# pinterest/rocksplicator

Hardware: AMD Instinct MI355X
Metric: replicated updates/sec (Put+Delete) at 1024 shards (higher is better)
Workload: dtype u8; 1 GPU; 1024shards_16Bkey_1024Bval_zipf0.99; key_len=16, val_len=1024, tick_updates=819200, parallelism=shard-parallel x1

## Files before the change

### rocksplicator_amd/csrc/engine.hip

```cpp
#include <hip/hip_runtime.h>

#define WB_UNALIGNED_OK 1

#include <algorithm>
#include <atomic>
#include <chrono>
#include <cstdio>
#include <cstring>
#include <deque>
#include <map>
#include <memory>
#include <mutex>
#include <string>
#include <thread>
#include <vector>

#include "../../include/rocksplicator_gpu.h"
#include "fold.h"
#include "host_store.h"
#include "part_copy.h"
#include "snappy.h"
#include "wb_format.h"

static thread_local std::string g_err;
extern "C" const char *gra_last_error(void) { return g_err.c_str(); }

#define HIP_TRY(x)                                                     \
  do {                                                                 \
    hipError_t _e = (x);                                               \
    if (_e != hipSuccess) {                                            \
      g_err = std::string(#x) + ": " + hipGetErrorString(_e);          \
      return GRA_ERR;                                                  \
    }                                                                  \
  } while (0)

namespace gra {

struct UpdDesc {
  uint64_t off;
  uint64_t base_seq;
  uint32_t len;
  uint32_t shard;
};
struct TickPlace {
  uint64_t cur;
  uint64_t hdr_off;
  uint64_t payload_off;
  uint64_t payload_bytes;
  uint32_t total_rec;
  uint32_t overflow;
};
struct SnapTask {
  uint64_t comp_off;
  uint64_t out_off;
  uint32_t comp_len;
  uint32_t ulen;
};
struct GroupDesc {
  uint32_t shard, first, n_upds, _pad;
};
struct DevRunDesc {
  uint64_t base_seq, last_seq;
  uint64_t cur;
  uint64_t hdr_off, payload_off;
  uint32_t n_entries, payload_bytes;
  uint32_t pay_rel_base;
  uint32_t shard;
};

__host__ __device__ inline uint2 add2(uint2 a, uint2 b) {
  return make_uint2(a.x + b.x, a.y + b.y);
}


constexpr uint32_t kSnapStage = 508;

__global__ void __launch_bounds__(256) k_snappy(
    const uint8_t *__restrict__ comp, const SnapTask *__restrict__ tasks,
    uint32_t n, uint8_t *__restrict__ scratch,
    uint32_t *__restrict__ err_ring, uint32_t tick) {
  __shared__ uint8_t lds[256 * (kSnapStage + 4)];
  uint32_t i = blockIdx.x * blockDim.x + threadIdx.x;
  if (i >= n) return;
  SnapTask t = tasks[i];
  uint8_t *dst = scratch + t.out_off;
  uint32_t r;
  if (t.comp_len <= kSnapStage) {
    uint8_t *mine = lds + threadIdx.x * (kSnapStage + 4);
    const uint8_t *src = comp + t.comp_off;
    for (uint32_t b = 0; b < t.comp_len; b += 16)
      *(uint4 *)(mine + b) = *(const uint4 *)(src + b);
    r = snp::decompress(mine, t.comp_len, dst, t.ulen);
  } else {
    r = snp::decompress(comp + t.comp_off, t.comp_len, dst, t.ulen);
  }
  if (r != t.ulen) {
    for (int b = 0; b < 13; b++) dst[b] = 0xFF;
    atomicAdd(&err_ring[tick % 64u], 1u);
  }
}

constexpr uint32_t kErrRing = 64;

constexpr uint32_t kRecCache = 2;

__device__ __forceinline__ uint2 block_scan256(uint2 v, uint2 *total) {
  __shared__ uint2 wsum[4];
  const uint32_t lane = threadIdx.x & 63u, w = threadIdx.x >> 6;
  uint2 inc = v;
  for (int ofs = 1; ofs < 64; ofs <<= 1) {
    uint32_t x = __shfl_up(inc.x, ofs, 64), y = __shfl_up(inc.y, ofs, 64);
    if (lane >= (uint32_t)ofs) inc = add2(inc, make_uint2(x, y));
  }
  if (lane == 63) wsum[w] = inc;
  __syncthreads();
  uint2 before = make_uint2(0, 0), tot = make_uint2(0, 0);
  for (uint32_t k = 0; k < 4; k++) {
    uint2 s = wsum[k];
    if (k < w) before = add2(before, s);
    tot = add2(tot, s);
  }
  *total = tot;
  return make_uint2(before.x + inc.x - v.x, before.y + inc.y - v.y);
}

__global__ void k_decode(const uint8_t *__restrict__ blobs,
                         const UpdDesc *__restrict__ descs, uint32_t n,
                         wb::WalkTotals *__restrict__ totals, uint32_t max_rec,
                         uint32_t *__restrict__ err_ring, uint32_t tick,
                         uint2 *__restrict__ partial, uint2 *__restrict__ bsums,
                         wb::Rec *__restrict__ reccache,
                         uint8_t *__restrict__ ok_out) {
  uint32_t i = blockIdx.x * 256 + threadIdx.x;
  uint2 v = make_uint2(0, 0);
  if (i < n) {
    UpdDesc d = descs[i];
    wb::Rec *cache = reccache + (size_t)i * kRecCache;
    wb::WalkTotals t = wb::walk_f(blobs + d.off, d.len,
                                  [&](const wb::Rec &r, uint32_t idx) {
                                    if (idx < kRecCache) cache[idx] = r;
                                  });
    if (t.n_records > max_rec) t.ok = 0;
    totals[i] = t;
    ok_out[i] = (uint8_t)t.ok;
    if (!t.ok) atomicAdd(&err_ring[tick % kErrRing], 1u);
    if (t.ok) v = make_uint2(t.n_records, t.payload16);
  }
  uint2 tot;
  uint2 excl = block_scan256(v, &tot);
  if (i < n) partial[i] = excl;
  if (threadIdx.x == 255) bsums[blockIdx.x] = tot;
}

__global__ void k_scan2(uint2 *__restrict__ bsums, uint32_t nblocks,
                        uint64_t *__restrict__ cursor,
                        TickPlace *__restrict__ place, uint64_t cap, int ring,
                        uint32_t task_cap, uint32_t *__restrict__ err_ring,
                        uint32_t tick) {
  const uint32_t per = (nblocks + 255) / 256;
  const uint32_t lo = threadIdx.x * per < nblocks ? threadIdx.x * per : nblocks;
  const uint32_t hi = lo + per < nblocks ? lo + per : nblocks;
  uint2 mine = make_uint2(0, 0);
  for (uint32_t i = lo; i < hi; i++) mine = add2(mine, bsums[i]);
  uint2 carry;
  uint2 run = block_scan256(mine, &carry);
  for (uint32_t i = lo; i < hi; i++) {
    uint2 v = bsums[i];
    bsums[i] = run;
    run = add2(run, v);
  }
  if (threadIdx.x == 0) {
    bsums[nblocks] = carry;
    uint2 tot = carry;
    uint64_t need_hdr = (((uint64_t)tot.x * sizeof(wb::RecHdr)) + 15) & ~15ULL;
    uint64_t need_pay = tot.y;
    uint64_t need = need_hdr + need_pay;
    TickPlace p = {};
    p.total_rec = tot.x;
    p.payload_bytes = need_pay;
    uint64_t cur = *cursor;
    if ((cur % cap) + need > cap) cur += cap - (cur % cap);
    if (need > cap || (!ring && cur + need > cap) ||
        (uint64_t)tot.x * 2 > task_cap) {
      p.overflow = 1;
      p.total_rec = 0;
      atomicAdd(&err_ring[tick % kErrRing], 1u);
    } else {
      p.cur = cur;
      p.hdr_off = cur % cap;
      p.payload_off = (cur % cap) + need_hdr;
      *cursor = cur + need;
    }
    *place = p;
    err_ring[(tick + kErrRing / 2) % kErrRing] = 0;
  }
}

__global__ void k_emit(const uint8_t *__restrict__ blobs,
                       const UpdDesc *__restrict__ descs, uint32_t n,
                       const wb::WalkTotals *__restrict__ totals,
                       const uint2 *__restrict__ partial,
                       const uint2 *__restrict__ bsums,
                       const TickPlace *__restrict__ place,
                       uint8_t *__restrict__ store,
                       CopyTask *__restrict__ tasks,
                       const wb::Rec *__restrict__ reccache) {
  uint32_t i = blockIdx.x * blockDim.x + threadIdx.x;
  if (i >= n) return;
  if (place->overflow) return;
  wb::WalkTotals t = totals[i];
  if (!t.ok || t.n_records == 0) return;
  UpdDesc d = descs[i];
  uint2 base = add2(partial[i], bsums[i >> 8]);
  wb::RecHdr *hdrs = (wb::RecHdr *)(store + place->hdr_off);
  uint8_t *pay_region = store + place->payload_off;
  uint32_t pay = base.y;
  uint32_t rec = base.x;
  auto emit_one = [&](const wb::Rec &r, uint32_t idx) {
    uint32_t cf4 = r.cf_id ? 4u : 0u;
    uint8_t btag = wb::base_tag(r.tag);
    uint32_t cfv = (cf4 && btag == wb::kRangeDeletion) ? 4u : 0u;
    wb::RecHdr h;
    h.seq = d.base_seq + idx;
    h.kv_off = pay;
    h.val_len = r.val_len + cfv;
    h.key_len = (uint16_t)(r.key_len + cf4);
    h.type = btag;
    h.flags = cf4 ? 1 : 0;
    h.kpref = 0;
    hdrs[rec + idx] = h;
    if (cf4) {
      *(uint32_t *)(pay_region + pay) = r.cf_id;
    }
    CopyTask tk;
    tk.src_off = d.off + r.key_off;
    tk.dst_rel = pay + cf4;
    tk.nbytes = r.key_len;
    tasks[2 * (rec + idx)] = tk;
    if (cfv) {
      uint8_t *p = pay_region + pay + cf4 + r.key_len;
      p[0] = (uint8_t)r.cf_id;
      p[1] = (uint8_t)(r.cf_id >> 8);
      p[2] = (uint8_t)(r.cf_id >> 16);
      p[3] = (uint8_t)(r.cf_id >> 24);
    }
    tk.src_off = d.off + r.val_off;
    tk.dst_rel = pay + cf4 + r.key_len + cfv;
    tk.nbytes = r.val_len;
    tasks[2 * (rec + idx) + 1] = tk;
    pay += (cf4 + r.key_len + cfv + r.val_len + 15u) & ~15u;
  };
  if (t.n_records <= kRecCache) {
    const wb::Rec *cache = reccache + (size_t)i * kRecCache;
    for (uint32_t idx = 0; idx < t.n_records; idx++) emit_one(cache[idx], idx);
  } else {
    wb::walk_f(blobs + d.off, d.len, emit_one);
  }
}

template <int G>
__device__ __forceinline__ void copy_dword(uint8_t *dst, const uint8_t *src,
                                           uint32_t n, uint32_t lane) {
  uint32_t head = (uint32_t)((0u - (uint32_t)(uintptr_t)dst) & 3u);
  if (head > n) head = n;
  if (lane < head) dst[lane] = src[lane];
  dst += head;
  src += head;
  n -= head;
  uint32_t nw = n >> 2;
  uint32_t r = (uint32_t)((uintptr_t)src & 3);
  const uint32_t *asrc = (const uint32_t *)(src - r);
  uint32_t *adst = (uint32_t *)dst;
  if (r == 0) {
    for (uint32_t w = lane; w < nw; w += G) adst[w] = asrc[w];
  } else {
    uint32_t sh = 8 * r;
    for (uint32_t w = lane; w < nw; w += G)
      adst[w] = (asrc[w] >> sh) | (asrc[w + 1] << (32 - sh));
  }
  uint32_t done = nw << 2, tail = n & 3;
  if (lane < tail) dst[done + lane] = src[done + lane];
}

template <int G, int R, bool UNAL>
__global__ void __launch_bounds__(256) k_copy(const uint8_t *__restrict__ blobs,
                                              uint8_t *__restrict__ store,
                                              const TickPlace *__restrict__ place,
                                              const CopyTask *__restrict__ tasks) {
  if (place->overflow) return;
  uint32_t wave = (blockIdx.x * blockDim.x + threadIdx.x) >> 6;
  uint32_t nwaves = (gridDim.x * blockDim.x) >> 6;
  pcopy::part_copy<G, R, UNAL>(blobs, store + place->payload_off, tasks,
                               place->total_rec, wave, nwaves);
}

__global__ void k_drain(const uint8_t *__restrict__ store,
                        const TickPlace *__restrict__ place,
                        uint8_t *__restrict__ hostbuf) {
  if (place->overflow) return;
  uint64_t hdr_bytes = (uint64_t)place->total_rec * sizeof(wb::RecHdr);
  uint64_t hb16 = (hdr_bytes + 15) & ~15ull;
  uint64_t pay = place->payload_bytes;
  const uint8_t *hsrc = store + place->hdr_off;
  const uint8_t *psrc = store + place->payload_off;
  size_t stride = (size_t)gridDim.x * blockDim.x * 16;
  size_t i0 = ((size_t)blockIdx.x * blockDim.x + threadIdx.x) * 16;
  for (size_t b = i0; b < hdr_bytes; b += stride)
    *(uint4 *)(hostbuf + b) = *(const uint4 *)(hsrc + b);
  uint8_t *pdst = hostbuf + hb16;
  for (size_t b = i0; b < pay; b += stride)
    *(uint4 *)(pdst + b) = *(const uint4 *)(psrc + b);
}

__global__ void k_rundesc(const GroupDesc *__restrict__ groups, uint32_t ngroups,
                          const UpdDesc *__restrict__ descs,
                          const wb::WalkTotals *__restrict__ totals,
                          const uint2 *__restrict__ partial,
                          const uint2 *__restrict__ bsums, uint32_t n,
                          uint32_t nblocks,
                          const TickPlace *__restrict__ place,
                          DevRunDesc *__restrict__ out) {
  uint32_t g = blockIdx.x * blockDim.x + threadIdx.x;
  if (g >= ngroups) return;
  GroupDesc gd = groups[g];
  auto scan_at = [&](uint32_t j) {
    return j >= n ? bsums[nblocks] : add2(partial[j], bsums[j >> 8]);
  };
  uint2 s0 = scan_at(gd.first);
  uint2 s1 = scan_at(gd.first + gd.n_upds);
  DevRunDesc rd = {};
  rd.shard = gd.shard;
  rd.n_entries = s1.x - s0.x;
  rd.payload_bytes = s1.y - s0.y;
  rd.pay_rel_base = s0.y;
  if (!place->overflow) {
    rd.cur = place->cur;
    rd.hdr_off = place->hdr_off + (uint64_t)s0.x * sizeof(wb::RecHdr);
    rd.payload_off = place->payload_off + s0.y;
    rd.base_seq = descs[gd.first].base_seq;
    const UpdDesc last = descs[gd.first + gd.n_upds - 1];
    rd.last_seq = last.base_seq + totals[gd.first + gd.n_upds - 1].hdr_count - 1;
  } else {
    rd.n_entries = 0;
  }
  out[g] = rd;
}

struct RunView {
  uint64_t hdr_off, payload_off;
  uint32_t n_entries, pay_rel_base;
};

__device__ inline int dev_memcmp(const uint8_t *a, const uint8_t *b, uint32_t n) {
  for (uint32_t i = 0; i < n; i++) {
    if (a[i] != b[i]) return a[i] < b[i] ? -1 : 1;
  }
  return 0;
}

struct MgExtra {
  uint64_t term_seq, merge_seq, rd_seq;
  uint32_t term_type, _pad;
};

__global__ void k_multiget(const uint8_t *__restrict__ store,
                           const RunView *__restrict__ runs, uint32_t nruns,
                           const GraKeyRef *__restrict__ keys,
                           const uint8_t *__restrict__ keybuf, uint32_t nq,
                           uint8_t *__restrict__ valbuf, uint32_t val_stride,
                           GraGetResult *__restrict__ out,
                           MgExtra *__restrict__ extra, int fold_u64) {
  __shared__ uint64_t sh_term_seq[256];
  __shared__ uint64_t sh_term_ref[256];
  __shared__ uint64_t sh_merge_seq[256];
  __shared__ uint64_t sh_rd_seq[256];
  uint32_t q = blockIdx.x;
  if (q >= nq) return;
  const uint8_t *key = keybuf + keys[q].off;
  uint32_t klen = keys[q].len;
  uint32_t qpref = wb::key_fnv_fold(wb::kFnvBasis32, key, klen);
  uint64_t term_seq = 0, term_ref = ~0ULL, merge_seq = 0, rd_seq = 0;
  for (uint32_t r = 0; r < nruns; r++) {
    RunView rv = runs[r];
    const wb::RecHdr *hdrs = (const wb::RecHdr *)(store + rv.hdr_off);
    const uint8_t *pay = store + rv.payload_off;
    for (uint32_t i = threadIdx.x; i < rv.n_entries; i += blockDim.x) {
      wb::RecHdr h = hdrs[i];
      if (h.type != wb::kRangeDeletion &&
          (h.key_len != klen || h.kpref != qpref))
        continue;
      uint32_t rel = h.kv_off - rv.pay_rel_base;
      if (h.type == wb::kRangeDeletion) {
        const uint8_t *b = pay + rel, *e2 = pay + rel + h.key_len;
        uint32_t bl = h.key_len, el = h.val_len;
        int c1 = dev_memcmp(b, key, bl < klen ? bl : klen);
        if (c1 > 0 || (c1 == 0 && bl > klen)) continue;
        int c2 = dev_memcmp(key, e2, klen < el ? klen : el);
        if (c2 > 0 || (c2 == 0 && klen >= el)) continue;
        if (h.seq > rd_seq) rd_seq = h.seq;
        continue;
      }
      if (dev_memcmp(pay + rel, key, klen) != 0)
        continue;
      if (h.type == wb::kMerge) {
        if (h.seq > merge_seq) merge_seq = h.seq;
      } else if (h.seq > term_seq) {
        term_seq = h.seq;
        term_ref = ((uint64_t)r << 32) | i;
      }
    }
  }
  uint32_t tid = threadIdx.x;
  sh_term_seq[tid] = term_seq;
  sh_term_ref[tid] = term_ref;
  sh_merge_seq[tid] = merge_seq;
  sh_rd_seq[tid] = rd_seq;
  __syncthreads();
  for (uint32_t ofs = blockDim.x / 2; ofs > 0; ofs >>= 1) {
    if (tid < ofs) {
      if (sh_term_seq[tid + ofs] > sh_term_seq[tid]) {
        sh_term_seq[tid] = sh_term_seq[tid + ofs];
        sh_term_ref[tid] = sh_term_ref[tid + ofs];
      }
      if (sh_merge_seq[tid + ofs] > sh_merge_seq[tid])
        sh_merge_seq[tid] = sh_merge_seq[tid + ofs];
      if (sh_rd_seq[tid + ofs] > sh_rd_seq[tid])
        sh_rd_seq[tid] = sh_rd_seq[tid + ofs];
    }
    __syncthreads();
  }
  uint64_t T = sh_term_seq[0], M = sh_merge_seq[0], RD = sh_rd_seq[0];
  uint64_t ref = sh_term_ref[0];
  uint8_t term_type = 0xFF;
  wb::RecHdr h = {};
  RunView rv = {};
  if (ref != ~0ULL) {
    rv = runs[ref >> 32];
    h = ((const wb::RecHdr *)(store + rv.hdr_off))[(uint32_t)ref];
    term_type = h.type;
  }
  if (tid == 0 && extra) {
    extra[q].term_seq = T;
    extra[q].merge_seq = M;
    extra[q].rd_seq = RD;
// ... 594 lines not shown
hipEvent_t GraEngine::get_event() {
  if (!event_pool.empty()) {
    hipEvent_t e = event_pool.back();
    event_pool.pop_back();
    return e;
  }
  hipEvent_t e;
  (void)hipEventCreate(&e);
  return e;
}
void GraEngine::put_event(hipEvent_t e) { event_pool.push_back(e); }

int GraEngine::init(const GraEngineOpts &o) {
  opts = o;
  if (opts.store_bytes == 0) opts.store_bytes = 4ULL << 30;
  if (opts.staging_bytes == 0) opts.staging_bytes = 256ULL << 20;
  if (opts.max_wb_records == 0) opts.max_wb_records = 1024;
  max_upd = 1u << 20;
  task_cap = 4u << 20;
  copy_grid = 2048;
  if (const char *g = getenv("GRA_COPY_GRID")) {
    long v = atol(g);
    copy_grid = (uint32_t)(v < 1 ? 1 : v > 2048 ? 2048 : v);
  }
  group_cap = opts.nshards + 1 > 65536 ? opts.nshards + 1 : 65536;
  (void)hipGetLastError();
  int ndev = 0;
  hipError_t de = hipGetDeviceCount(&ndev);
  if (de != hipSuccess || ndev == 0) {
    g_err = "no HIP device present — the GPU apply path refuses to run "
            "(no CPU fallback by design)";
    return GRA_NO_GPU;
  }
  if (opts.device >= 0) {
    hipError_t se = hipSetDevice(opts.device);
    if (se != hipSuccess) {
      g_err = std::string("hipSetDevice: ") + hipGetErrorString(se);
      (void)hipGetLastError();
      return GRA_ERR;
    }
  }
  HIP_TRY(hipStreamCreate(&stream));
  HIP_TRY(hipStreamCreate(&copyout));
  HIP_TRY(hipStreamCreate(&h2d));
  HIP_TRY(hipStreamCreate(&prep));
  HIP_TRY(hipMalloc(&d_store, opts.store_bytes + 16));
  HIP_TRY(hipMalloc(&d_cursor, 8));
  HIP_TRY(hipMemset(d_cursor, 0, 8));
  HIP_TRY(hipMalloc(&d_totals, (size_t)max_upd * sizeof(wb::WalkTotals)));
  HIP_TRY(hipMalloc(&d_partial, (size_t)max_upd * sizeof(uint2)));
  HIP_TRY(hipMalloc(&d_bsums, ((size_t)max_upd / 256 + 2) * sizeof(uint2)));
  HIP_TRY(hipMalloc(&d_reccache, (size_t)max_upd * 2 * sizeof(wb::Rec)));
  HIP_TRY(hipMalloc(&d_tasks, (size_t)task_cap * sizeof(CopyTask)));
  HIP_TRY(hipMalloc(&d_place, kSlots * sizeof(TickPlace)));
  HIP_TRY(hipMalloc(&d_groups, (size_t)group_cap * sizeof(GroupDesc)));
  HIP_TRY(hipMalloc(&d_err_ring, kErrRing * 4));
  HIP_TRY(hipMemset(d_err_ring, 0, kErrRing * 4));
  for (int i = 0; i < 2; i++) {
    HIP_TRY(hipMalloc(&d_stage_blobs_bufs[i], opts.staging_bytes + 16));
    HIP_TRY(hipMalloc(&d_stage_descs_bufs[i], (size_t)max_upd * sizeof(UpdDesc)));
    HIP_TRY(hipEventCreate(&stage_used_ev[i]));
    HIP_TRY(hipEventRecord(stage_used_ev[i], stream));
    HIP_TRY(hipEventCreateWithFlags(&h2d_gate_ev[i], hipEventDisableTiming));
    HIP_TRY(hipEventRecord(h2d_gate_ev[i], h2d));
  }
  static std::atomic<uint64_t> g_epoch{1};
  for (int i = 0; i < 2; i++) {
    HIP_TRY(hipHostMalloc(&stage[i].pin, opts.staging_bytes + 16,
                          hipHostMallocNonCoherent));
    stage[i].descs = (GraUpdateDesc *)malloc((size_t)max_upd * sizeof(GraUpdateDesc));
    stage[i].epoch = g_epoch.fetch_add(1u << 20);
    HIP_TRY(hipEventCreate(&stage[i].free_ev));
    HIP_TRY(hipEventRecord(stage[i].free_ev, stream));
  }
  cur_stage.store(&stage[0]);
  for (int i = 0; i < kSlots; i++) {
    Slot &s = slots[i];
    HIP_TRY(hipHostMalloc(&s.h_groups, (size_t)group_cap * sizeof(GroupDesc)));
    HIP_TRY(hipHostMalloc(&s.h_place, sizeof(TickPlace)));
    HIP_TRY(hipHostMalloc(&s.h_rundescs, (size_t)group_cap * sizeof(DevRunDesc)));
    HIP_TRY(hipMalloc(&s.d_rundescs, (size_t)group_cap * sizeof(DevRunDesc)));
    HIP_TRY(hipMalloc(&s.d_ok, (size_t)max_upd));
    HIP_TRY(hipHostMalloc(&s.h_ok, (size_t)max_upd));
    HIP_TRY(hipHostMalloc(&s.h_err, 4));
    HIP_TRY(hipHostMalloc(&s.h_descs, (size_t)max_upd * sizeof(UpdDesc)));
  }
  if (opts.drain_host && opts.store_ring &&
      opts.store_bytes < 10 * opts.staging_bytes) {
    g_err = "drain_host with store_ring needs store_bytes >= 10x "
            "staging_bytes (ring wrap inside the drain pipeline)";
    return GRA_ERR;
  }
  shards = std::vector<ShardState>(opts.nshards);
  event_pool.reserve(kSlots * kEventsPerTick);
  for (int i = 0; i < kSlots * kEventsPerTick; i++) {
    hipEvent_t ev;
    HIP_TRY(hipEventCreate(&ev));
    event_pool.push_back(ev);
  }
  return GRA_OK;
}

GraEngine::~GraEngine() {
  {
    std::lock_guard<std::mutex> lk(drain_mu);
    closing = true;
  }
  (void)hipStreamSynchronize(stream);
  (void)hipStreamSynchronize(copyout);
  (void)hipStreamSynchronize(h2d);
  for (auto &t : pending)
    for (int i = 0; i < kEventsPerTick; i++)
      if (t.ev[i]) (void)hipEventDestroy(t.ev[i]);
  for (auto e : event_pool) (void)hipEventDestroy(e);
  for (int i = 0; i < 2; i++) {
    if (stage[i].pin) (void)hipHostFree(stage[i].pin);
    free(stage[i].descs);
    if (stage[i].free_ev) (void)hipEventDestroy(stage[i].free_ev);
  }
  for (int i = 0; i < kSlots; i++) {
    Slot &s = slots[i];
    if (s.h_groups) (void)hipHostFree(s.h_groups);
    if (s.h_place) (void)hipHostFree(s.h_place);
    if (s.h_rundescs) (void)hipHostFree(s.h_rundescs);
    if (s.d_rundescs) (void)hipFree(s.d_rundescs);
    if (s.d_ok) (void)hipFree(s.d_ok);
    if (s.h_ok) (void)hipHostFree(s.h_ok);
    if (s.h_err) (void)hipHostFree(s.h_err);
    if (s.h_descs) (void)hipHostFree(s.h_descs);
  }
  for (void *p : {(void *)mg.d_runs, (void *)mg.d_keys, (void *)mg.d_keybuf,
                  (void *)mg.d_valbuf, (void *)mg.d_out, mg.d_extra,
                  mg.d_qtab, mg.d_cands, mg.d_tombs, mg.d_aux,
                  (void *)mg.d_counts})
    if (p) (void)hipFree(p);
  if (mg.h_counts) (void)hipHostFree(mg.h_counts);
  for (void *p : {(void *)sc.d_runs, (void *)sc.d_bounds, (void *)sc.d_out,
                  (void *)sc.d_cands, (void *)sc.d_tombs, (void *)sc.d_items,
                  (void *)sc.d_bsums, (void *)sc.d_ents, (void *)sc.d_ctl,
                  (void *)sc.d_heads, (void *)sc.d_folds, (void *)sc.d_cp})
    if (p) (void)hipFree(p);
  if (sc.h_ctl) (void)hipHostFree(sc.h_ctl);
  if (sc.h_cp) (void)hipHostFree(sc.h_cp);
  for (int i = 0; i < 2; i++) {
    if (d_stage_blobs_bufs[i]) (void)hipFree(d_stage_blobs_bufs[i]);
    if (d_stage_descs_bufs[i]) (void)hipFree(d_stage_descs_bufs[i]);
    if (stage_used_ev[i]) (void)hipEventDestroy(stage_used_ev[i]);
    if (h2d_gate_ev[i]) (void)hipEventDestroy(h2d_gate_ev[i]);
  }
  for (void *p : {(void *)d_totals, (void *)d_partial, (void *)d_bsums,
                  (void *)d_reccache, (void *)d_store, (void *)d_cursor,
                  (void *)d_tasks,
                  (void *)d_place, (void *)d_groups, (void *)d_err_ring})
    if (p) (void)hipFree(p);
  shards.clear();
  pending.clear();
  {
    std::lock_guard<std::mutex> lk(drain_mu);
    for (auto &pr : drain_pool) (void)hipHostFree(pr.first);
    drain_pool.clear();
  }
  if (stream) (void)hipStreamDestroy(stream);
  if (copyout) (void)hipStreamDestroy(copyout);
  if (h2d) (void)hipStreamDestroy(h2d);
  if (prep) (void)hipStreamDestroy(prep);
}

int GraEngine::free_slot() {
  for (;;) {
    for (int i = 0; i < kSlots; i++)
      if (!slots[i].busy) return i;
    int rc = ingest(false);
    if (rc != GRA_OK) return -1;
    if (!pending.empty()) {
      if (ingest_one(pending.front(), true) != GRA_OK) return -1;
      pending.pop_front();
    }
  }
}

int GraEngine::enqueue_tick(TickInput &in) {
  const uint32_t n = in.n;
  const uint64_t blob_bytes = in.blob_bytes;
  const std::vector<GroupDesc> &groups = *in.groups;
  if (n == 0) return GRA_OK;
  if (n > max_upd) {
    g_err = "tick exceeds max updates per tick";
    return GRA_ERR;
  }
  if (opts.drain_host && opts.store_ring && blob_bytes * 10 > opts.store_bytes) {
    g_err = "drain_host with store_ring needs store_bytes >= 10x the tick "
            "size (ring wrap inside the drain pipeline)";
    return GRA_ERR;
  }
  if (groups.size() > group_cap) {
    g_err = "tick exceeds max shard-groups per tick";
    return GRA_ERR;
  }
  int si = free_slot();
  if (si < 0) return GRA_ERR;
  Slot &sl = slots[si];
  sl.busy = true;
  uint32_t ngroups = (uint32_t)groups.size();
  memcpy(sl.h_groups, groups.data(), ngroups * sizeof(GroupDesc));
  const GroupDesc *groups_for_kernel = in.d_groups ? in.d_groups : d_groups;
  uint32_t tick = tick_id++;

  TickRec t;
  t.slot = si;
  t.n = n;
  t.ngroups = ngroups;
  t.blob_bytes = blob_bytes;
  t.counts = std::move(in.counts);
  for (int i = 0; i < kEventsPerTick; i++) t.ev[i] = get_event();
  static const bool detailed = env_flag("GRA_DETAILED_EVENTS");

  if (!in.d_groups) {
    HIP_TRY(hipMemcpyAsync(d_groups, sl.h_groups, ngroups * sizeof(GroupDesc),
                           hipMemcpyHostToDevice, stream));
  }
  HIP_TRY(t.record(kEvTickStart, stream));
  const uint8_t *d_blobs = in.d_blobs;
  const UpdDesc *d_descw = in.d_descs;
  int stage_buf = -1;
  if (in.stage_src != nullptr) {
    stage_buf = (int)(tick & 1u);
    d_blobs = d_stage_blobs_bufs[stage_buf];
    if (in.h_descs) d_descw = d_stage_descs_bufs[stage_buf];
    HIP_TRY(hipEventSynchronize(h2d_gate_ev[stage_buf]));
    HIP_TRY(hipStreamWaitEvent(h2d, stage_used_ev[stage_buf], 0));
    HIP_TRY(t.record(kEvH2dStart, h2d));
    HIP_TRY(hipMemcpyAsync(d_stage_blobs_bufs[stage_buf], in.stage_src,
                           in.stage_bytes, hipMemcpyHostToDevice, h2d));
    if (in.h_descs) {
      memcpy(sl.h_descs, in.h_descs, (size_t)n * sizeof(UpdDesc));
      HIP_TRY(hipMemcpyAsync(d_stage_descs_bufs[stage_buf], sl.h_descs,
                             (size_t)n * sizeof(UpdDesc),
                             hipMemcpyHostToDevice, h2d));
    }
    HIP_TRY(t.record(kEvH2dDone, h2d));
    HIP_TRY(hipEventRecord(h2d_gate_ev[stage_buf], h2d));
    HIP_TRY(hipStreamWaitEvent(stream, t.ev[kEvH2dDone], 0));
  }
  uint32_t nb = (n + 255) / 256;
  if (in.d_snaptasks) {
    if (in.window_ev) HIP_TRY(hipStreamWaitEvent(prep, in.window_ev, 0));
    HIP_TRY(t.record(kEvSnappyStart, prep));
    hipLaunchKernelGGL(k_snappy, dim3(nb), dim3(256), 0, prep, in.d_comp,
                       in.d_snaptasks, n, (uint8_t *)d_blobs, d_err_ring,
                       tick);
    HIP_TRY(hipGetLastError());
    HIP_TRY(t.record(kEvSnappyDone, prep));
    HIP_TRY(hipStreamWaitEvent(stream, t.ev[kEvSnappyDone], 0));
  }
  hipLaunchKernelGGL(k_decode, dim3(nb), dim3(256), 0, stream, d_blobs,
                     d_descw, n, d_totals, opts.max_wb_records, d_err_ring,
                     tick, d_partial, d_bsums, d_reccache, sl.d_ok);
  HIP_TRY(hipGetLastError());
  if (detailed) HIP_TRY(t.record(kEvAfterDecode, stream));
  TickPlace *place_slot = d_place + si;
  hipLaunchKernelGGL(k_scan2, dim3(1), dim3(256), 0, stream, d_bsums, nb,
                     d_cursor, place_slot, opts.store_bytes, opts.store_ring,
                     task_cap, d_err_ring, tick);
  HIP_TRY(hipGetLastError());
  if (detailed) HIP_TRY(t.record(kEvAfterScan, stream));
  hipLaunchKernelGGL(k_emit, dim3(nb), dim3(256), 0, stream, d_blobs, d_descw,
                     n, d_totals, d_partial, d_bsums, place_slot, d_store,
                     d_tasks, d_reccache);
  HIP_TRY(hipGetLastError());
  HIP_TRY(t.record(kEvAfterEmit, stream));
  {
    const size_t avg = blob_bytes / n;
    const dim3 grid(copy_grid), blk(256);
    if (avg >= 768)
      hipLaunchKernelGGL((k_copy<64, 4, false>), grid, blk, 0, stream, d_blobs,
                         d_store, place_slot, d_tasks);
    else if (avg >= 384)
      hipLaunchKernelGGL((k_copy<32, 4, true>), grid, blk, 0, stream, d_blobs,
                         d_store, place_slot, d_tasks);
    else if (avg >= 192)
      hipLaunchKernelGGL((k_copy<16, 4, true>), grid, blk, 0, stream, d_blobs,
                         d_store, place_slot, d_tasks);
    else
      hipLaunchKernelGGL((k_copy<8, 4, true>), grid, blk, 0, stream, d_blobs,
                         d_store, place_slot, d_tasks);
  }
  HIP_TRY(hipGetLastError());
  HIP_TRY(t.record(kEvAfterCopy, stream));
  if (in.window_ev)
    HIP_TRY(hipEventRecord(in.window_ev, stream));
  hipLaunchKernelGGL(k_rundesc, dim3((ngroups + 255) / 256), dim3(256), 0,
                     stream, groups_for_kernel, ngroups, d_descw, d_totals,
                     d_partial, d_bsums, n, nb, place_slot, sl.d_rundescs);
  HIP_TRY(hipGetLastError());
  HIP_TRY(t.record(kEvMainEnd, stream));
  if (stage_buf >= 0)
    HIP_TRY(hipEventRecord(stage_used_ev[stage_buf], stream));
  HIP_TRY(hipStreamWaitEvent(copyout, t.ev[kEvMainEnd], 0));
  HIP_TRY(hipMemcpyAsync(sl.h_rundescs, sl.d_rundescs,
                         (size_t)ngroups * sizeof(DevRunDesc),
                         hipMemcpyDeviceToHost, copyout));
  HIP_TRY(hipMemcpyAsync(sl.h_err, d_err_ring + (tick % kErrRing), 4,
                         hipMemcpyDeviceToHost, copyout));
  HIP_TRY(hipMemcpyAsync(sl.h_ok, sl.d_ok, n, hipMemcpyDeviceToHost, copyout));
  HIP_TRY(hipMemcpyAsync(sl.h_place, place_slot, sizeof(TickPlace),
                         hipMemcpyDeviceToHost, copyout));
  if (opts.drain_host && !t.counts.empty()) {
    uint64_t recs = 0;
    for (uint32_t c : t.counts) recs += c;
    size_t need = (size_t)blob_bytes + 46 * recs + 80;
    t.drain_buf = drain_alloc(need);
    if (t.drain_buf) {
      hipLaunchKernelGGL(k_drain, dim3(1024), dim3(256), 0, copyout, d_store,
                         place_slot, t.drain_buf.get());
      HIP_TRY(hipGetLastError());
    }
  }
  HIP_TRY(t.record(kEvPublished, copyout));
  pending.push_back(std::move(t));
  return GRA_OK;
}

static int fetch_run_impl(GraEngine *e, Run &r);

static std::shared_ptr<Run> run_from(const DevRunDesc &rd, bool on_device) {
  auto run = std::make_shared<Run>();
  run->base_seq = rd.base_seq;
  run->last_seq = rd.last_seq;
  run->n_entries = rd.n_entries;
  run->payload_bytes = rd.payload_bytes;
  run->pay_rel_base = rd.pay_rel_base;
  if (on_device) {
    run->hdr_cur = rd.hdr_off;
    run->payload_cur = rd.payload_off;
  }
  return run;
}

static void roll_back_locked(ShardState &ss) {
  ss.next_seq = ss.durable_seq + 1;
  while (!ss.log.empty() && ss.log.back().base_seq > ss.durable_seq) {
    ss.log_used -= ss.log.back().rep.size();
    ss.log.pop_back();
  }
}

int GraEngine::ingest_one(TickRec &t, bool wait) {
  if (wait) {
    HIP_TRY(hipEventSynchronize(t.ev[kEvPublished]));
  } else {
    hipError_t q = hipEventQuery(t.ev[kEvPublished]);
    if (q == hipErrorNotReady) return GRA_NOT_FOUND;
    if (q != hipSuccess) {
      g_err = std::string("tick event: ") + hipGetErrorString(q);
      return GRA_ERR;
    }
  }
  Slot &sl = slots[t.slot];
  float ms;
  auto dt = [&](TickEvent a, TickEvent b) {
    if (!t.has(a) || !t.has(b)) return 0.0;
    (void)hipEventElapsedTime(&ms, t.ev[a], t.ev[b]);
    return (double)ms;
  };
  stats.h2d_ms += dt(kEvH2dStart, kEvH2dDone);
  stats.snappy_ms += dt(kEvSnappyStart, kEvSnappyDone);
  TickEvent prev = t.has(kEvH2dDone) ? kEvH2dDone : kEvTickStart;
  if (t.has(kEvAfterDecode)) {
    stats.decode_ms += dt(prev, kEvAfterDecode);
    prev = kEvAfterDecode;
  }
  if (t.has(kEvAfterScan)) {
    stats.scan_ms += dt(prev, kEvAfterScan);
    prev = kEvAfterScan;
  }
  stats.emit_ms += dt(prev, kEvAfterEmit);
  stats.copy_ms += dt(kEvAfterEmit, kEvAfterCopy);
  stats.runfix_ms += dt(kEvAfterCopy, kEvMainEnd);
  stats.total_ms += dt(kEvTickStart, kEvMainEnd);
  stats.ticks += 1;
  stats.updates += t.n;
  stats.blob_bytes += t.blob_bytes;
  uint32_t err = *sl.h_err;
  auto attach_drain = [&](Run &run, const DevRunDesc &rd) -> bool {
    if (!t.drain_buf || sl.h_place->overflow) return false;
    uint64_t hb16 =
        ((uint64_t)sl.h_place->total_rec * sizeof(wb::RecHdr) + 15) & ~15ull;
    run.hbuf = t.drain_buf;
    run.hdr_p = t.drain_buf.get() + (rd.hdr_off - sl.h_place->hdr_off);
    run.pay_p = t.drain_buf.get() + hb16;
    return true;
  };
  if (err != 0) {
    const bool have_counts = t.counts.size() == t.n;
    for (uint32_t g = 0; g < t.ngroups; g++) {
      DevRunDesc &rd = sl.h_rundescs[g];
      const GroupDesc &gd = sl.h_groups[g];
      ShardState &ss = shards[rd.shard];
      std::lock_guard<std::mutex> lk(ss.mu);
      if (rd.base_seq == 0) {
        ss.poisoned = true;
        ss.cnt_failures++;
        roll_back_locked(ss);
        continue;
      }
      if (ss.poisoned) {
        roll_back_locked(ss);
        continue;
      }
      uint32_t keep_recs = 0;
      uint64_t keep_seq = rd.base_seq - 1;
      bool bad = false;
      for (uint32_t i = 0; i < gd.n_upds; i++) {
        if (!sl.h_ok[gd.first + i]) {
          bad = true;
          break;
        }
        uint32_t c = have_counts ? t.counts[gd.first + i] : 0;
        keep_recs += c;
        keep_seq += c;
      }
      if (!bad) {
        auto run = run_from(rd, true);
        if (opts.drain_host && !attach_drain(*run, rd))
          (void)fetch_run_impl(this, *run);
        if (rd.n_entries > 0 && !opts.store_ring) ss.runs.push_back(std::move(run));
        if (rd.last_seq > ss.durable_seq) ss.durable_seq = rd.last_seq;
        stats.records += rd.n_entries;
        stats.payload_bytes += rd.payload_bytes;
        continue;
      }
      if (keep_recs > 0 && have_counts && !opts.store_ring) {
        auto run = run_from(rd, true);
        run->last_seq = keep_seq;
        run->n_entries = keep_recs;
        if (opts.drain_host && !attach_drain(*run, rd))
          (void)fetch_run_impl(this, *run);
        ss.runs.push_back(std::move(run));
        stats.records += keep_recs;
      }
      if (keep_seq > ss.durable_seq) ss.durable_seq = keep_seq;
      ss.poisoned = true;
      ss.cnt_failures++;
      roll_back_locked(ss);
    }
  } else if (opts.store_ring) {
    for (uint32_t g = 0; g < t.ngroups; g++) {
      DevRunDesc &rd = sl.h_rundescs[g];
      ShardState &ss = shards[rd.shard];
      std::lock_guard<std::mutex> lk(ss.mu);
      if (ss.poisoned) {
        roll_back_locked(ss);
        continue;
      }
      if (opts.drain_host && rd.n_entries > 0) {
        auto run = run_from(rd, false);
        if (attach_drain(*run, rd)) ss.runs.push_back(std::move(run));
      }
      if (rd.last_seq > ss.durable_seq) ss.durable_seq = rd.last_seq;
      stats.records += rd.n_entries;
      stats.payload_bytes += rd.payload_bytes;
    }
  } else {
    for (uint32_t g = 0; g < t.ngroups; g++) {
      DevRunDesc &rd = sl.h_rundescs[g];
      ShardState &ss = shards[rd.shard];
      std::lock_guard<std::mutex> lk(ss.mu);
      if (ss.poisoned) {
        roll_back_locked(ss);
        continue;
      }
      if (rd.n_entries > 0) {
        auto run = run_from(rd, true);
        if (opts.drain_host && !attach_drain(*run, rd))
          (void)fetch_run_impl(this, *run);
        ss.runs.push_back(std::move(run));
      }
      if (rd.last_seq > ss.durable_seq) ss.durable_seq = rd.last_seq;
      stats.records += rd.n_entries;
      stats.payload_bytes += rd.payload_bytes;
    }
  }
  for (int i = 0; i < kEventsPerTick; i++) put_event(t.ev[i]);
  sl.busy = false;
  return GRA_OK;
}

int GraEngine::ingest(bool wait_all) {
  while (!pending.empty()) {
    int rc = ingest_one(pending.front(), wait_all);
    if (rc == GRA_NOT_FOUND) return GRA_OK;
    if (rc != GRA_OK) return rc;
    pending.pop_front();
  }
  return GRA_OK;
}

int GraEngine::stream_tick_locked() {
  StageBuf *old = cur_stage.load(std::memory_order_acquire);
  if (old->nslots.load(std::memory_order_relaxed) == 0) return GRA_OK;
  StageBuf *next = old == &stage[0] ? &stage[1] : &stage[0];
  HIP_TRY(hipEventSynchronize(next->free_ev));
  next->pos.store(0, std::memory_order_relaxed);
  next->nslots.store(0, std::memory_order_relaxed);
  next->staged.store(0, std::memory_order_relaxed);
  next->epoch++;
  next->closed.store(false, std::memory_order_release);
  old->closed.store(true, std::memory_order_seq_cst);
  cur_stage.store(next, std::memory_order_release);
  for (int s = 0; s < kWriterSlots; s++)
    while (old->writers[s].n.load(std::memory_order_seq_cst) != 0)
      std::this_thread::yield();
  uint32_t nall = old->nslots.load(std::memory_order_relaxed);
  if (nall > max_upd) nall = max_upd;
  uint64_t fill = old->pos.load(std::memory_order_relaxed);
  if (fill > opts.staging_bytes) fill = opts.staging_bytes;
  std::vector<uint32_t> cnt(opts.nshards + 1, 0);
  for (uint32_t i = 0; i < nall; i++)
    if (old->descs[i].len) cnt[old->descs[i].shard + 1]++;
  for (uint32_t s = 0; s < opts.nshards; s++) cnt[s + 1] += cnt[s];
  uint32_t n = cnt[opts.nshards];
  if (gra_check_staging()) {
    uint32_t expect = old->staged.load(std::memory_order_relaxed);
    if (n != expect)
      fprintf(stderr,
              "[gra] BUG: tick build found %u staged updates, expected %u\n",
              n, expect);
  }
  if (n == 0) return GRA_OK;
  std::vector<UpdDesc> ud(n);
  std::vector<GroupDesc> groups;
  uint64_t blob_bytes = 0;
  {
    std::vector<uint32_t> pos = cnt;
    for (uint32_t i = 0; i < nall; i++) {
      const GraUpdateDesc &d = old->descs[i];
      if (!d.len) continue;
      uint32_t j = pos[d.shard]++;
      ud[j].off = d.off;
      ud[j].len = d.len;
      ud[j].shard = d.shard;
      ud[j].base_seq = (uint64_t)d.ts;
      blob_bytes += d.len;
    }
    for (uint32_t s = 0; s < opts.nshards; s++)
      if (cnt[s + 1] > cnt[s])
        groups.push_back({s, cnt[s], cnt[s + 1] - cnt[s], 0});
  }
  TickInput in;
  in.n = n;
  in.groups = &groups;
  in.blob_bytes = blob_bytes;
  in.counts.resize(n);
  for (uint32_t i = 0; i < n; i++)
    in.counts[i] = wb::fixed32_le(old->pin + ud[i].off + 8);
  in.stage_src = old->pin;
  in.stage_bytes = fill;
  in.h_descs = ud.data();
  int rc = enqueue_tick(in);
  if (rc != GRA_OK) return rc;
  HIP_TRY(hipEventRecord(old->free_ev, h2d));
  return GRA_OK;
}

int GraEngine::flush_locked() {
  int rc = stream_tick_locked();
  if (rc != GRA_OK) return rc;
  HIP_TRY(hipStreamSynchronize(stream));
  return ingest(true);
}

extern "C" {

void gra_engine_opts_init(GraEngineOpts *o) {
  memset(o, 0, sizeof(*o));
  o->device = -1;
  o->nshards = 1;
}

int gra_engine_create(const GraEngineOpts *opts, GraEngine **out) {
  auto *e = new GraEngine();
  int rc = e->init(*opts);
  if (rc != GRA_OK) {
    delete e;
    return rc;
  }
  *out = e;
  return GRA_OK;
}

void gra_engine_destroy(GraEngine *e) { delete e; }

GraDb *gra_open(GraEngine *e, uint32_t shard) {
  if (shard >= e->opts.nshards) {
    g_err = "shard id out of range";
    return nullptr;
  }
  return new GraDb{e, shard};
}
void gra_close(GraDb *db) { delete db; }

static void retain_locked(GraEngine *e, ShardState &ss, uint64_t base_seq,
                          uint32_t count, int64_t ts, const uint8_t *rep,
                          size_t len) {
  uint64_t per_shard = (e->opts.log_bytes ? e->opts.log_bytes : 256ULL << 20) /
                       (e->opts.nshards ? e->opts.nshards : 1);
  LogEnt ent;
  ent.base_seq = base_seq;
  ent.count = count;
  ent.ts = ts;
  ent.rep.assign(rep, rep + len);
  ss.log_used += len;
  ss.log.push_back(std::move(ent));
  while (ss.log_used > per_shard && ss.log.size() > 1) {
    ss.log_used -= ss.log.front().rep.size();
    ss.log.pop_front();
  }
}

int gra_handle_replicate_response(GraDb *db, const uint8_t *rep, size_t len,
                                  int64_t ts) {
  GraEngine *e = db->e;
  ShardState &ss = e->shards[db->shard];
  uint64_t base;
  uint32_t count;
  bool was_poisoned = false;
  {
    std::lock_guard<std::mutex> lk(ss.mu);
    if (ss.poisoned) {
      was_poisoned = true;
    } else {
      if (len < wb::kHeaderBytes) return 0;
      count = wb::fixed32_le(rep + 8);
      base = ss.next_seq;
      ss.next_seq += count;
    }
  }
  if (was_poisoned) {
    {
      std::lock_guard<std::mutex> lk(e->mu);
      (void)e->flush_locked();
    }
    std::lock_guard<std::mutex> lk(ss.mu);
    ss.poisoned = false;
    return 0;
  }
  auto rollback = [&] {
    std::lock_guard<std::mutex> lk(ss.mu);
    if (ss.next_seq == base + count) ss.next_seq = base;
  };
  if (len + 16 > e->opts.staging_bytes) {
    rollback();
    return 0;
  }
  struct Chunk {
    GraEngine *e = nullptr;
    GraEngine::StageBuf *sb = nullptr;
    uint64_t epoch = 0;
    uint64_t base = 0, used = 0, cap = 0;
    uint32_t slot = 0, slots_left = 0;
  };
  thread_local Chunk ck;
  constexpr uint64_t kChunkBytes = 256 << 10;
  static std::atomic<uint32_t> g_wslot{0};
  thread_local const uint32_t wslot =
      g_wslot.fetch_add(1, std::memory_order_relaxed) %
      GraEngine::kWriterSlots;
  bool staged = false;
  for (int attempt = 0; attempt < 100000 && !staged; attempt++) {
    GraEngine::StageBuf *sb = e->cur_stage.load(std::memory_order_acquire);
    auto &w = sb->writers[wslot].n;
    w.fetch_add(1, std::memory_order_seq_cst);
    if (sb->closed.load(std::memory_order_seq_cst)) {
      w.fetch_sub(1, std::memory_order_acq_rel);
      std::this_thread::yield();
      continue;
    }
    bool chunk_ok = ck.e == e && ck.sb == sb && ck.epoch == sb->epoch &&
                    ck.used + len <= ck.cap && ck.slots_left > 0;
    if (!chunk_ok) {
      uint64_t want = len > kChunkBytes ? (uint64_t)len : kChunkBytes;
      uint32_t cslots = (uint32_t)(want / (len ? len : 1)) + 8;
      if (cslots > 4096) cslots = 4096;
      uint64_t off = sb->pos.fetch_add(want, std::memory_order_relaxed);
      uint32_t slot = sb->nslots.fetch_add(cslots, std::memory_order_relaxed);
      if (off + want + 16 > e->opts.staging_bytes ||
          slot + cslots > e->max_upd) {
        for (uint32_t i = slot; i < slot + cslots && i < e->max_upd; i++)
          sb->descs[i].len = 0;
        ck.sb = nullptr;
        w.fetch_sub(1, std::memory_order_acq_rel);
        if (e->cur_stage.load(std::memory_order_acquire) == sb) {
          std::lock_guard<std::mutex> lk(e->mu);
          if (e->cur_stage.load(std::memory_order_acquire) == sb) {
            if (e->stream_tick_locked() != GRA_OK) {
              rollback();
// ... 1300 lines not shown
```

### rocksplicator_amd/csrc/wb_format.h

```cpp
#pragma once
#include <stdint.h>

#ifdef __HIP__
#define WB_HD __host__ __device__ inline
#define WB_HD_OP __host__ __device__
#else
#define WB_HD static inline
#define WB_HD_OP
#endif

namespace wb {

enum Tag : uint8_t {
  kDeletion = 0x00,
  kValue = 0x01,
  kMerge = 0x02,
  kLogData = 0x03,
  kCfDeletion = 0x04,
  kCfValue = 0x05,
  kCfMerge = 0x06,
  kSingleDeletion = 0x07,
  kCfSingleDeletion = 0x08,
  kBeginPrepare = 0x09,
  kEndPrepare = 0x0A,
  kCommit = 0x0B,
  kRollback = 0x0C,
  kNoop = 0x0D,
  kCfRangeDeletion = 0x0E,
  kRangeDeletion = 0x0F,
  kMaxTag = 0x0F,
};

constexpr uint32_t kHeaderBytes = 12;

WB_HD uint64_t fixed64_le(const uint8_t *p) {
#if defined(__HIP_DEVICE_COMPILE__) && defined(WB_UNALIGNED_OK)
  return *(const uint64_t *)p;
#else
  uint64_t v = 0;
  for (int i = 0; i < 8; i++) v |= (uint64_t)p[i] << (8 * i);
  return v;
#endif
}
WB_HD uint32_t fixed32_le(const uint8_t *p) {
#if defined(__HIP_DEVICE_COMPILE__) && defined(WB_UNALIGNED_OK)
  return *(const uint32_t *)p;
#else
  return (uint32_t)p[0] | ((uint32_t)p[1] << 8) | ((uint32_t)p[2] << 16) |
         ((uint32_t)p[3] << 24);
#endif
}

WB_HD uint32_t varint32(const uint8_t *p, uint32_t avail, uint32_t *out) {
  uint32_t result = 0;
#pragma unroll
  for (uint32_t i = 0; i < 5; i++) {
    if (i >= avail) return 0;
    uint32_t byte = p[i];
    if (byte & 0x80) {
      result |= (byte & 0x7F) << (7 * i);
    } else {
      if (i == 4 && byte > 0x0F) return 0;
      result |= byte << (7 * i);
      *out = result;
      return i + 1;
    }
  }
  return 0;
}

constexpr uint32_t kFnvBasis32 = 2166136261u;
WB_HD uint32_t key_fnv_fold(uint32_t h, const uint8_t *p, uint32_t n) {
  for (uint32_t i = 0; i < n; i++) h = (h ^ p[i]) * 16777619u;
  return h;
}

WB_HD bool consumes_seq(uint8_t tag) {
  switch (tag) {
    case kValue: case kDeletion: case kMerge: case kSingleDeletion:
    case kRangeDeletion: case kCfValue: case kCfDeletion: case kCfMerge:
    case kCfSingleDeletion: case kCfRangeDeletion:
      return true;
    default:
      return false;
  }
}
WB_HD bool has_cf_prefix(uint8_t tag) {
  return tag == kCfValue || tag == kCfDeletion || tag == kCfMerge ||
         tag == kCfSingleDeletion || tag == kCfRangeDeletion;
}
WB_HD uint8_t base_tag(uint8_t tag) {
  switch (tag) {
    case kCfValue: return kValue;
    case kCfDeletion: return kDeletion;
    case kCfMerge: return kMerge;
    case kCfSingleDeletion: return kSingleDeletion;
    case kCfRangeDeletion: return kRangeDeletion;
    default: return tag;
  }
}
WB_HD int nslices(uint8_t btag) {
  switch (btag) {
    case kValue: case kMerge: case kRangeDeletion: return 2;
    case kDeletion: case kSingleDeletion: return 1;
    case kLogData: return 2 - 1;
    case kEndPrepare: case kCommit: case kRollback: return 1;
    case kBeginPrepare: case kNoop: return 0;
    default: return -1;
  }
}

struct Rec {
  uint32_t key_off, key_len;
  uint32_t val_off, val_len;
  uint8_t tag;
  uint8_t consumes;
  uint16_t _pad;
  uint32_t cf_id;
};

struct WalkTotals {
  uint32_t n_records;
  uint32_t payload_bytes;
  uint32_t payload16;
  uint32_t hdr_count;
  uint32_t ok;
  uint32_t _pad;
  uint64_t hdr_seq;
};

template <class F>
WB_HD WalkTotals walk_f(const uint8_t *rep, uint32_t len, F &&f) {
  WalkTotals t = {0, 0, 0, 0, 0, 0, 0};
  if (len < kHeaderBytes) return t;
  t.hdr_seq = fixed64_le(rep);
  t.hdr_count = fixed32_le(rep + 8);
  uint32_t pos = kHeaderBytes;
  uint32_t consumed = 0, nrec = 0, payload = 0, payload16 = 0;
  while (pos < len) {
    uint8_t tag = rep[pos++];
    uint8_t bt = base_tag(tag);
    int ns = nslices(bt);
    if (ns < 0) return t;
    uint32_t cf = 0;
    if (has_cf_prefix(tag)) {
      uint32_t c = varint32(rep + pos, len - pos, &cf);
      if (c == 0) return t;
      pos += c;
    }
    uint32_t off[2] = {0, 0}, slen[2] = {0, 0};
    for (int s = 0; s < ns; s++) {
      uint32_t n, c = varint32(rep + pos, len - pos, &n);
      if (c == 0) return t;
      pos += c;
      if (pos + n > len || n > len) return t;
      off[s] = pos;
      slen[s] = n;
      pos += n;
    }
    if (consumes_seq(tag)) {
      Rec r;
      r.key_off = off[0];
      r.key_len = slen[0];
      r.val_off = off[1];
      r.val_len = slen[1];
      r.tag = tag;
      r.consumes = 1;
      r._pad = 0;
      r.cf_id = cf;
      f(r, nrec);
      uint32_t cf4 = cf ? 4u : 0u;
      uint32_t cfx = (cf && bt == kRangeDeletion) ? 8u : cf4;
      payload += slen[0] + slen[1] + cfx;
      payload16 += (slen[0] + slen[1] + cfx + 15u) & ~15u;
      nrec++;
      consumed++;
    }
  }
  if (consumed != t.hdr_count) return t;
  t.n_records = nrec;
  t.payload_bytes = payload;
  t.payload16 = payload16;
  t.ok = 1;
  return t;
}

struct NullEmit {
  WB_HD_OP void operator()(const Rec &, uint32_t) const {}
};

WB_HD WalkTotals walk(const uint8_t *rep, uint32_t len, Rec *emit, uint32_t cap) {
  if (!emit) return walk_f(rep, len, NullEmit{});
  return walk_f(rep, len, [&](const Rec &r, uint32_t i) {
    if (i < cap) emit[i] = r;
  });
}

struct RecHdr {
  uint64_t seq;
  uint32_t kv_off;
  uint32_t val_len;
  uint16_t key_len;
  uint8_t type;
  uint8_t flags;
  uint32_t kpref;
};

WB_HD uint32_t key_prefix4(const uint8_t *key, uint32_t klen) {
  uint32_t p = 0;
  for (uint32_t i = 0; i < 4 && i < klen; i++) p |= (uint32_t)key[i] << (8 * i);
  return p;
}
static_assert(sizeof(RecHdr) == 24, "RecHdr must be 24 bytes");

}
```

Baseline: 1.813 billion updates/s.

## Stage write-batch headers in LDS for decode and fetch ok flags only on error

The decode kernel now loads the first 48 bytes of each write batch with 16-byte vector loads into a per-thread shared-memory row, and the walker reads bytes from that window before falling back to global memory. This replaces scattered byte-wise global loads for the header and first record tags and varints. Separately, the per-tick device-to-host copy of the ok array is dropped and done synchronously only when the error counter is nonzero. The costs are extra LDS use (about 13 KB per block), which may limit occupancy, plus a branch on every byte access.

```diff
diff --git a/rocksplicator_amd/csrc/engine.hip b/rocksplicator_amd/csrc/engine.hip
--- a/rocksplicator_amd/csrc/engine.hip
+++ b/rocksplicator_amd/csrc/engine.hip
@@ -124,22 +124,42 @@
   return make_uint2(before.x + inc.x - v.x, before.y + inc.y - v.y);
 }
 
-__global__ void k_decode(const uint8_t *__restrict__ blobs,
-                         const UpdDesc *__restrict__ descs, uint32_t n,
-                         wb::WalkTotals *__restrict__ totals, uint32_t max_rec,
-                         uint32_t *__restrict__ err_ring, uint32_t tick,
-                         uint2 *__restrict__ partial, uint2 *__restrict__ bsums,
-                         wb::Rec *__restrict__ reccache,
-                         uint8_t *__restrict__ ok_out) {
+constexpr uint32_t kDecodeWin = 48;
+static_assert(kDecodeWin % 16 == 0, "window is staged in 16 B chunks");
+
+__global__ void __launch_bounds__(256) k_decode(
+    const uint8_t *__restrict__ blobs, const UpdDesc *__restrict__ descs,
+    uint32_t n, wb::WalkTotals *__restrict__ totals, uint32_t max_rec,
+    uint32_t *__restrict__ err_ring, uint32_t tick,
+    uint2 *__restrict__ partial, uint2 *__restrict__ bsums,
+    wb::Rec *__restrict__ reccache, uint8_t *__restrict__ ok_out) {
+  __shared__ uint32_t stage[256 * (kDecodeWin + 4) / 4];
   uint32_t i = blockIdx.x * 256 + threadIdx.x;
   uint2 v = make_uint2(0, 0);
   if (i < n) {
     UpdDesc d = descs[i];
+    const uint8_t *rep = blobs + d.off;
+    uint32_t *row = stage + threadIdx.x * ((kDecodeWin + 4) / 4);
+    const uint32_t nch = wb::win_chunks(d.len, kDecodeWin);
+    uint4 c[kDecodeWin / 16];
+#pragma unroll
+    for (uint32_t k = 0; k < kDecodeWin / 16; k++)
+      if (k < nch) c[k] = *(const uint4 *)(rep + 16 * k);
+#pragma unroll
+    for (uint32_t k = 0; k < kDecodeWin / 16; k++)
+      if (k < nch) {
+        row[4 * k + 0] = c[k].x;
+        row[4 * k + 1] = c[k].y;
+        row[4 * k + 2] = c[k].z;
+        row[4 * k + 3] = c[k].w;
+      }
+    wb::WinSrc src = {(const uint8_t *)row, wb::win_bytes(d.len, kDecodeWin),
+                      rep};
     wb::Rec *cache = reccache + (size_t)i * kRecCache;
-    wb::WalkTotals t = wb::walk_f(blobs + d.off, d.len,
-                                  [&](const wb::Rec &r, uint32_t idx) {
-                                    if (idx < kRecCache) cache[idx] = r;
-                                  });
+    wb::WalkTotals t = wb::walk_src(src, d.len,
+                                    [&](const wb::Rec &r, uint32_t idx) {
+                                      if (idx < kRecCache) cache[idx] = r;
+                                    });
     if (t.n_records > max_rec) t.ok = 0;
     totals[i] = t;
     ok_out[i] = (uint8_t)t.ok;
@@ -1340,7 +1360,6 @@
                          hipMemcpyDeviceToHost, copyout));
   HIP_TRY(hipMemcpyAsync(sl.h_err, d_err_ring + (tick % kErrRing), 4,
                          hipMemcpyDeviceToHost, copyout));
-  HIP_TRY(hipMemcpyAsync(sl.h_ok, sl.d_ok, n, hipMemcpyDeviceToHost, copyout));
   HIP_TRY(hipMemcpyAsync(sl.h_place, place_slot, sizeof(TickPlace),
                          hipMemcpyDeviceToHost, copyout));
   if (opts.drain_host && !t.counts.empty()) {
@@ -1430,6 +1449,7 @@
     return true;
   };
   if (err != 0) {
+    HIP_TRY(hipMemcpy(sl.h_ok, sl.d_ok, t.n, hipMemcpyDeviceToHost));
     const bool have_counts = t.counts.size() == t.n;
     for (uint32_t g = 0; g < t.ngroups; g++) {
       DevRunDesc &rd = sl.h_rundescs[g];
diff --git a/rocksplicator_amd/csrc/wb_format.h b/rocksplicator_amd/csrc/wb_format.h
--- a/rocksplicator_amd/csrc/wb_format.h
+++ b/rocksplicator_amd/csrc/wb_format.h
@@ -51,12 +51,47 @@
 #endif
 }
 
-WB_HD uint32_t varint32(const uint8_t *p, uint32_t avail, uint32_t *out) {
+struct PtrSrc {
+  const uint8_t *p;
+  WB_HD_OP uint8_t byte(uint32_t pos) const { return p[pos]; }
+  WB_HD_OP uint32_t u32(uint32_t pos) const { return fixed32_le(p + pos); }
+  WB_HD_OP uint64_t u64(uint32_t pos) const { return fixed64_le(p + pos); }
+};
+
+struct WinSrc {
+  const uint8_t *win;
+  uint32_t win_len;
+  const uint8_t *rep;
+  WB_HD_OP uint8_t byte(uint32_t pos) const {
+    return pos < win_len ? win[pos] : rep[pos];
+  }
+  WB_HD_OP uint32_t u32(uint32_t pos) const {
+    if (pos + 4 > win_len) return fixed32_le(rep + pos);
+#if defined(__HIP_DEVICE_COMPILE__)
+    if ((pos & 3u) == 0) return *(const uint32_t *)(win + pos);
+#endif
+    return (uint32_t)win[pos] | ((uint32_t)win[pos + 1] << 8) |
+           ((uint32_t)win[pos + 2] << 16) | ((uint32_t)win[pos + 3] << 24);
+  }
+  WB_HD_OP uint64_t u64(uint32_t pos) const {
+    if (pos + 8 > win_len) return fixed64_le(rep + pos);
+    return (uint64_t)u32(pos) | ((uint64_t)u32(pos + 4) << 32);
+  }
+};
+
+WB_HD uint32_t win_bytes(uint32_t len, uint32_t W) { return len < W ? len : W; }
+WB_HD uint32_t win_chunks(uint32_t len, uint32_t W) {
+  return (win_bytes(len, W) + 15u) / 16u;
+}
+
+template <class Src>
+WB_HD uint32_t varint32_src(const Src &src, uint32_t pos, uint32_t avail,
+                            uint32_t *out) {
   uint32_t result = 0;
 #pragma unroll
   for (uint32_t i = 0; i < 5; i++) {
     if (i >= avail) return 0;
-    uint32_t byte = p[i];
+    uint32_t byte = src.byte(pos + i);
     if (byte & 0x80) {
       result |= (byte & 0x7F) << (7 * i);
     } else {
@@ -67,6 +102,9 @@
     }
   }
   return 0;
+}
+WB_HD uint32_t varint32(const uint8_t *p, uint32_t avail, uint32_t *out) {
+  return varint32_src(PtrSrc{p}, 0, avail, out);
 }
 
 constexpr uint32_t kFnvBasis32 = 2166136261u;
@@ -129,28 +167,28 @@
   uint64_t hdr_seq;
 };
 
-template <class F>
-WB_HD WalkTotals walk_f(const uint8_t *rep, uint32_t len, F &&f) {
+template <class Src, class F>
+WB_HD WalkTotals walk_src(const Src &src, uint32_t len, F &&f) {
   WalkTotals t = {0, 0, 0, 0, 0, 0, 0};
   if (len < kHeaderBytes) return t;
-  t.hdr_seq = fixed64_le(rep);
-  t.hdr_count = fixed32_le(rep + 8);
+  t.hdr_seq = src.u64(0);
+  t.hdr_count = src.u32(8);
   uint32_t pos = kHeaderBytes;
   uint32_t consumed = 0, nrec = 0, payload = 0, payload16 = 0;
   while (pos < len) {
-    uint8_t tag = rep[pos++];
+    uint8_t tag = src.byte(pos++);
     uint8_t bt = base_tag(tag);
     int ns = nslices(bt);
     if (ns < 0) return t;
     uint32_t cf = 0;
     if (has_cf_prefix(tag)) {
-      uint32_t c = varint32(rep + pos, len - pos, &cf);
+      uint32_t c = varint32_src(src, pos, len - pos, &cf);
       if (c == 0) return t;
       pos += c;
     }
     uint32_t off[2] = {0, 0}, slen[2] = {0, 0};
     for (int s = 0; s < ns; s++) {
-      uint32_t n, c = varint32(rep + pos, len - pos, &n);
+      uint32_t n, c = varint32_src(src, pos, len - pos, &n);
       if (c == 0) return t;
       pos += c;
       if (pos + n > len || n > len) return t;
@@ -185,6 +223,11 @@
   return t;
 }
 
+template <class F>
+WB_HD WalkTotals walk_f(const uint8_t *rep, uint32_t len, F &&f) {
+  return walk_src(PtrSrc{rep}, len, f);
+}
+
 struct NullEmit {
   WB_HD_OP void operator()(const Rec &, uint32_t) const {}
 };
```

New measurement: 1.869 billion updates/s, median of 6. +3.1%, better.
